# eleurent/rl-agents

Hardware: AMD Instinct MI355X
Metric: rollout env-steps/sec (UCT plan(), budget=1000) (higher is better)
Workload: dtype f64; 1 GPU; uct_highway_shaped_S10000_A5_budget1000_e33xh30_roots262144_per_gpu; n_roots_per_gpu=262144, n_roots_total=262144, states=10000, actions=5, episodes=33, horizon=30, parallelism=roots sharded over 1 GPU(s)

## Files before the change

rl_agents_amd/csrc/api.hip:

```cpp
#include <dlfcn.h>
#include <math.h>
#include <stdarg.h>
#include <stdlib.h>
#include <string.h>

#include <algorithm>
#include <mutex>
#include <set>
#include <unordered_map>
#include <vector>

#include "common.hpp"
#include "each_host.hpp"
#include "libm_sincos.hpp"
#include "seed_sequence.hpp"

namespace mp {

thread_local std::string g_err;

int fail(int code, const char *fmt, ...)
{
    char buf[1024];
    va_list ap;
    va_start(ap, fmt);
    vsnprintf(buf, sizeof(buf), fmt, ap);
    va_end(ap);
    g_err = buf;
    return code;
}

int ws_reserve(mp_ctx *ctx, int slot, size_t bytes, void **out)
{
    DevBuf &b = ctx->ws[slot];
    if (bytes > b.cap) {
        if (b.p) {
            MP_HIP(hipStreamSynchronize(ctx->stream));
            MP_HIP(hipFree(b.p));
// ... 102 lines not shown
    uint64_t k = (uint64_t)key;
    out[0] = (uint32_t)k;
    if (!(k >> 32)) return 1;
    out[1] = (uint32_t)(k >> 32);
    return 2;
}
}

__global__ void pack_records(int S, int A, const int32_t *__restrict__ T, const double *__restrict__ R,
                             const uint8_t *__restrict__ term, const uint8_t *__restrict__ avail, Rec *__restrict__ rec)
{
    const long i = (long)blockIdx.x * blockDim.x + threadIdx.x;
    if (i >= (long)S * A) return;
    const int s = (int)(i / A);
    Rec r;
    r.next = T[i];
    r.flags = (term && term[s] ? 1u : 0u) | (term && term[r.next] ? 2u : 0u) | (!avail || avail[i] ? 4u : 0u);
    r.reward = R[i];
    rec[i] = r;
}

__global__ void pack_records_range(int s0, int ns, int A, const int32_t *__restrict__ T, const double *__restrict__ R,
                                   const uint8_t *__restrict__ term, const uint8_t *__restrict__ avail, Rec *__restrict__ rec,
                                   uint16_t *__restrict__ t16)
{
    const long j = (long)blockIdx.x * blockDim.x + threadIdx.x;
    if (j >= (long)ns * A) return;
    const long i = (long)s0 * A + j;
    const int s = (int)(i / A);
    Rec r;
    r.next = T[i];
    r.flags = (term && term[s] ? 1u : 0u) | (term && term[r.next] ? 2u : 0u) | (!avail || avail[i] ? 4u : 0u);
    r.reward = R[i];
    rec[i] = r;
    if (t16) t16[i] = (uint16_t)((uint32_t)r.next | (term && term[r.next] ? 0x8000u : 0u));
}

__global__ void pack_joint_range(int first, int count, int M, int Sb, int A, long S, const int32_t *__restrict__ t_new,
                                 const double *__restrict__ r_new, const uint8_t *__restrict__ term_new,
                                 const uint8_t *__restrict__ avail, int32_t *__restrict__ T, double *__restrict__ R,
                                 uint8_t *__restrict__ term_all, Rec *__restrict__ rec_all)
{
    const long j = (long)blockIdx.x * blockDim.x + threadIdx.x;
    const long sa = (long)Sb * A;
    if (j >= (long)count * M * sa) return;
    const int cm = (int)(j / sa);
    const int c = cm / M, m = cm - c * M;
    const int sl = (int)((j - (long)cm * sa) / A), a = (int)(j - (long)cm * sa - (long)sl * A);
    const int base = (first + c) * Sb;
    const long i = ((long)m * S + base + sl) * A + a;
    const int nl = t_new[j];
    const uint8_t *tm = term_new ? term_new + (long)cm * Sb : nullptr;
    Rec r;
    r.next = base + nl;
    r.flags = (tm && tm[sl] ? 1u : 0u) | (tm && tm[nl] ? 2u : 0u) | (!avail || avail[i] ? 4u : 0u);
    r.reward = r_new[j];
    T[i] = r.next;
    R[i] = r.reward;
    rec_all[i] = r;
    if (a == 0 && tm) term_all[(long)m * S + base + sl] = tm[sl];
}

__global__ void scatter_rows(int n_rows, int A, const int32_t *__restrict__ rows, const int32_t *__restrict__ t_new,
                             const double *__restrict__ r_new, const uint8_t *__restrict__ term_new,
                             const uint8_t *__restrict__ r8_new, int32_t *__restrict__ T, double *__restrict__ R,
                             uint8_t *__restrict__ term, uint8_t *__restrict__ r8)
{
    const long j = (long)blockIdx.x * blockDim.x + threadIdx.x;
    if (j >= (long)n_rows * A) return;
    const int k = (int)(j / A), a = (int)(j - (long)k * A);
    const long i = (long)rows[k] * A + a;
    T[i] = t_new[j];
    R[i] = r_new[j];
    if (r8 && r8_new) r8[i] = r8_new[j];
    if (a == 0 && term && term_new) term[rows[k]] = term_new[k];
}

__global__ void pack_records_rows(int n_rows, int A, const int32_t *__restrict__ rows, const int32_t *__restrict__ T,
                                  const double *__restrict__ R, const uint8_t *__restrict__ term, const uint8_t *__restrict__ avail,
                                  Rec *__restrict__ rec, uint16_t *__restrict__ t16)
{
    const long j = (long)blockIdx.x * blockDim.x + threadIdx.x;
    if (j >= (long)n_rows * A) return;
    const int k = (int)(j / A), a = (int)(j - (long)k * A);
    const int s = rows[k];
    const long i = (long)s * A + a;
    Rec r;
    r.next = T[i];
    r.flags = (term && term[s] ? 1u : 0u) | (term && term[r.next] ? 2u : 0u) | (!avail || avail[i] ? 4u : 0u);
    r.reward = R[i];
    rec[i] = r;
    if (t16) t16[i] = (uint16_t)((uint32_t)r.next | (term && term[r.next] ? 0x8000u : 0u));
}

__global__ void globalize_roots(int n, int Sb, int NB, const int32_t *__restrict__ model_index, const int32_t *__restrict__ local,
                                int32_t *__restrict__ global, int32_t *__restrict__ fault)
{
    const int i = blockIdx.x * blockDim.x + threadIdx.x;
    if (i >= n) return;
    const int m = model_index[i], s = local[i];
    const bool bad = m < 0 || m >= NB || s < 0 || s >= Sb;
    if (bad && fault) atomicAdd(fault, 1);
    global[i] = bad ? 0 : m * Sb + s;
}

__global__ void globalize_joint_roots(int n, int M, int Sb, int NB, const int32_t *__restrict__ model_index,
                                      const int32_t *__restrict__ local, int32_t *__restrict__ global, int32_t *__restrict__ fault)
{
    const int i = blockIdx.x * blockDim.x + threadIdx.x;
    if (i >= n) return;
    const int b = model_index[i];
    bool bad = b < 0 || b >= NB;
    for (int m = 0; m < M; ++m) {
        const int s = local[(long)i * M + m];
        bad |= s < 0 || s >= Sb;
// ... 665 lines not shown
{
    const size_t n = (size_t)M * S * A;
    MP_HIP(hipSetDevice(ctx->device));
    mp_model *m = new mp_model();
    m->ctx = ctx; m->mode = MP_MODE_DETERMINISTIC; m->M = M; m->S = S; m->A = A; m->Sc = S; m->NB = 1; m->Sb = S;
    m->done_on_next = done_on_next ? 1 : 0; m->max_steps = max_steps > 0 ? max_steps : 0;
    auto bail = [&](int rc) { mp_model_free(m); return rc; };
    if (hipMalloc(&m->T, n * sizeof(int32_t)) != hipSuccess || hipMalloc(&m->R, n * sizeof(double)) != hipSuccess ||
        hipMalloc(&m->rec, (size_t)S * A * sizeof(Rec)) != hipSuccess)
        return bail(fail(MP_ERR_ALLOC, "mp_model_load_table: hipMalloc failed"));
    if (terminal && hipMalloc(&m->term, (size_t)S) != hipSuccess) return bail(fail(MP_ERR_ALLOC, "hipMalloc failed"));
    if (hipMemcpy(m->T, t32.data(), n * sizeof(int32_t), hipMemcpyHostToDevice) != hipSuccess ||
        hipMemcpy(m->R, reward, n * sizeof(double), hipMemcpyHostToDevice) != hipSuccess ||
        (terminal && hipMemcpy(m->term, terminal, (size_t)S, hipMemcpyHostToDevice) != hipSuccess))
        return bail(fail(MP_ERR_HIP, "mp_model_load_table: upload failed"));
    const long sa = (long)S * A;
    hipLaunchKernelGGL(pack_records, dim3((unsigned)((sa + 255) / 256)), dim3(256), 0, ctx->stream, S, A, m->T, m->R,
                       m->term, (const uint8_t *)nullptr, m->rec);
    if (S < 32768) {
        if (hipMalloc(&m->t16, (((size_t)sa * 2 + 15) & ~(size_t)15) + 16) != hipSuccess)
            return bail(fail(MP_ERR_ALLOC, "mp_model_load_table: hipMalloc failed"));
        hipLaunchKernelGGL(pack_t16, dim3((unsigned)((sa + 255) / 256)), dim3(256), 0, ctx->stream, S, A, m->T, m->term,
                           m->t16);
        m->rmap = new std::unordered_map<uint64_t, int>();
        std::unordered_map<uint64_t, int> &seen = *m->rmap;
        std::vector<uint8_t> idx(((size_t)sa + 15) & ~(size_t)15, 0);
        std::vector<double> dict(256, 0.0);
        bool fits = true;
        for (long i = 0; i < sa && fits; ++i) {
            uint64_t bits;
            memcpy(&bits, &reward[i], sizeof(bits));
            auto it = seen.find(bits);
            if (it == seen.end()) {
                if (seen.size() == 256) { fits = false; break; }
                it = seen.emplace(bits, (int)seen.size()).first;
                dict[it->second] = reward[i];
            }
            idx[i] = (uint8_t)it->second;
        }
        if (fits) {
            if (hipMalloc(&m->r8, idx.size()) != hipSuccess || hipMalloc(&m->rdict, 256 * sizeof(double)) != hipSuccess)
                return bail(fail(MP_ERR_ALLOC, "mp_model_load_table: hipMalloc failed"));
            if (hipMemcpy(m->r8, idx.data(), idx.size(), hipMemcpyHostToDevice) != hipSuccess ||
                hipMemcpy(m->rdict, dict.data(), 256 * sizeof(double), hipMemcpyHostToDevice) != hipSuccess)
                return bail(fail(MP_ERR_HIP, "mp_model_load_table: upload failed"));
            m->n_rdict = (int)seen.size();
// ... 151 lines not shown
        for (size_t i = 0; i < n && keep_compact; ++i) {
            const int k = reward_index(m, reward[i], &grew);
            if (k < 0) keep_compact = false;
            else idx[i] = (uint8_t)k;
        }
    }
    hipStream_t s = ctx->stream;
    const size_t g0 = (size_t)first * Sb;
    MP_HIP(hipMemcpyAsync(m->T + g0 * A, t32, n * 4, hipMemcpyHostToDevice, s));
    MP_HIP(hipMemcpyAsync(m->R + g0 * A, st + off_r, n * 8, hipMemcpyHostToDevice, s));
    if (terminal) MP_HIP(hipMemcpyAsync(m->term + g0, st + off_term, ns, hipMemcpyHostToDevice, s));
    if (compact && keep_compact) {
        MP_HIP(hipMemcpyAsync(m->r8 + g0 * A, st + off_r8, n, hipMemcpyHostToDevice, s));
        if (grew) {
            double *dict = reinterpret_cast<double *>(st + off_dict);
            for (const auto &kv : *m->rmap) memcpy(&dict[kv.second], &kv.first, 8);
            MP_HIP(hipMemcpyAsync(m->rdict, dict, m->rmap->size() * 8, hipMemcpyHostToDevice, s));
            m->n_rdict = (int)m->rmap->size();
        }
    } else if (compact) {
        drop_compact_rewards(m);
    }
    hipLaunchKernelGGL(pack_records_range, dim3((unsigned)((n + 255) / 256)), dim3(256), 0, s, (int)g0, (int)ns, A, m->T, m->R,
                       m->term, (const uint8_t *)m->avail, m->rec, m->t16);
    MP_HIP(hipGetLastError());
    MP_HIP(hipEventRecord(m->upd_done, s));
    m->upd_pending = true;
    m->serial = mp::next_model_serial();
    return MP_OK;
}

int mp_model_update_rows(mp_model *m, int32_t n_rows, const int32_t *rows, const int64_t *transition, const double *reward,
                         const uint8_t *terminal)
{
    if (!m || !rows || !transition || !reward) return fail(MP_ERR_ARG, "mp_model_update_rows: NULL argument");
    if (m->mode != MP_MODE_DETERMINISTIC || !m->rec || m->M != 1 || m->rec_all)
        return fail(MP_ERR_MODE, "mp_model_update_rows: deterministic table models (M = 1) only");
    if (n_rows < 1) return fail(MP_ERR_ARG, "mp_model_update_rows: n_rows = %d", n_rows);
    if (terminal && !m->term) return fail(MP_ERR_ARG, "mp_model_update_rows: the model was loaded without terminal flags");
    const int Sb = m->Sb > 0 ? m->Sb : m->S, A = m->A;
    mp_ctx *ctx = m->ctx;
    MP_HIP(hipSetDevice(ctx->device));
    const size_t n = (size_t)n_rows * A;
    const bool compact = m->r8 && m->rmap && m->n_rdict > 0;
    const size_t off_t = ((size_t)n_rows * 4 + 15) & ~(size_t)15, off_r = (off_t + n * 4 + 15) & ~(size_t)15, off_term = off_r + n * 8,
                 off_r8 = (off_term + n_rows + 15) & ~(size_t)15, off_dict = (off_r8 + n + 15) & ~(size_t)15, total = off_dict + 256 * 8;
    MP_TRY(update_blocks(m, total, total));
// ... 24 lines not shown
            else idx[i] = (uint8_t)k;
        }
    }
    if (compact && keep_compact && grew) {
        double *dict = reinterpret_cast<double *>(st + off_dict);
        for (const auto &kv : *m->rmap) memcpy(&dict[kv.second], &kv.first, 8);
    }
    hipStream_t s = ctx->stream;
    char *dv = static_cast<char *>(m->upd_dev);
    MP_HIP(hipMemcpyAsync(dv, st, total, hipMemcpyHostToDevice, s));
    if (compact && keep_compact && grew) {
        MP_HIP(hipMemcpyAsync(m->rdict, dv + off_dict, m->rmap->size() * 8, hipMemcpyDeviceToDevice, s));
        m->n_rdict = (int)m->rmap->size();
    }
    if (compact && !keep_compact) drop_compact_rewards(m);
    const int32_t *drows = reinterpret_cast<const int32_t *>(dv);
    hipLaunchKernelGGL(scatter_rows, dim3((unsigned)((n + 255) / 256)), dim3(256), 0, s, n_rows, A, drows,
                       reinterpret_cast<const int32_t *>(dv + off_t), reinterpret_cast<const double *>(dv + off_r),
                       terminal ? reinterpret_cast<const uint8_t *>(dv + off_term) : (const uint8_t *)nullptr,
                       compact && keep_compact ? reinterpret_cast<const uint8_t *>(dv + off_r8) : (const uint8_t *)nullptr, m->T, m->R,
                       m->term, compact && keep_compact ? m->r8 : (uint8_t *)nullptr);
    if (!terminal) {
        hipLaunchKernelGGL(pack_records_rows, dim3((unsigned)((n + 255) / 256)), dim3(256), 0, s, n_rows, A, drows, m->T, m->R, m->term,
                           (const uint8_t *)m->avail, m->rec, m->t16);
    } else {
        std::sort(owners.begin(), owners.end());
        owners.erase(std::unique(owners.begin(), owners.end()), owners.end());
        if (owners.size() > 64) {
            const long sa = (long)m->S * A;
            hipLaunchKernelGGL(pack_records_range, dim3((unsigned)((sa + 255) / 256)), dim3(256), 0, s, 0, m->S, A, m->T, m->R, m->term,
                               (const uint8_t *)m->avail, m->rec, m->t16);
        } else {
            const long sa = (long)Sb * A;
            for (int32_t b : owners)
                hipLaunchKernelGGL(pack_records_range, dim3((unsigned)((sa + 255) / 256)), dim3(256), 0, s, b * Sb, Sb, A, m->T, m->R,
                                   m->term, (const uint8_t *)m->avail, m->rec, m->t16);
        }
    }
    MP_HIP(hipGetLastError());
    MP_HIP(hipEventRecord(m->upd_done, s));
    m->upd_pending = true;
    m->serial = mp::next_model_serial();
    return MP_OK;
}

int mp_model_load_joint(mp_ctx *ctx, int32_t M, int32_t S, int32_t A, const int64_t *transition, const double *reward,
                        const uint8_t *terminal, int32_t done_on_next, mp_model **out)
{
    if (!ctx || !out || !transition || !reward) return fail(MP_ERR_ARG, "mp_model_load_joint: NULL argument");
    MP_TRY(mp_model_load_table(ctx, M, S, A, transition, reward, terminal, done_on_next, 0, out));
    mp_model *m = *out;
    auto bail = [&](int rc) { mp_model_free(m); *out = nullptr; return rc; };
    const long sa = (long)S * A;
    if (hipMalloc(&m->rec_all, (size_t)M * sa * sizeof(Rec)) != hipSuccess) return bail(fail(MP_ERR_ALLOC, "mp_model_load_joint: hipMalloc failed"));
    if (terminal) {
        if (hipMalloc(&m->term_all, (size_t)M * S) != hipSuccess) return bail(fail(MP_ERR_ALLOC, "mp_model_load_joint: hipMalloc failed"));
        if (hipMemcpy(m->term_all, terminal, (size_t)M * S, hipMemcpyHostToDevice) != hipSuccess)
            return bail(fail(MP_ERR_HIP, "mp_model_load_joint: upload failed"));
    }
// ... 313 lines not shown
    mp_model *m = new mp_model();
    m->ctx = ctx; m->mode = MP_MODE_CARTPOLE; m->M = 1; m->S = 0; m->A = 2;
    m->cp_sincos = mp_libm_sincos_variant();
    if (const char *e = getenv("MP_CARTPOLE_SINCOS"))
        m->cp_sincos = !strcmp(e, "fma") ? SINCOS_LIBM_FMA : (!strcmp(e, "plain") ? SINCOS_LIBM_PLAIN : SINCOS_DEVICE);
    m->cp = *params;
    m->max_steps = params->max_steps;
    *out = m;
    return MP_OK;
}

int mp_model_free(mp_model *m)
{
    if (!m) return MP_OK;
    if (m->ctx) hipSetDevice(m->ctx->device);
    if (!m->borrowed) {
        if (m->P) hipFree(const_cast<double *>(m->P));
        if (m->R) hipFree(m->R);
        if (m->term && m->term != m->term_all) hipFree(m->term);
    }
    if (m->T) hipFree(m->T);
    if (m->rec && m->rec != m->rec_all) hipFree(m->rec);
    if (m->t16) hipFree(m->t16);
    if (m->r8) hipFree(m->r8);
    if (m->rdict) hipFree(m->rdict);
    if (m->sa_cost) hipFree(m->sa_cost);
    if (m->avail) hipFree(m->avail);
    if (m->rec_all) hipFree(m->rec_all);
    if (m->term_all) hipFree(m->term_all);
    if (m->NXT) hipFree(m->NXT);
    if (m->thr) hipFree(m->thr);
    if (m->srec) hipFree(m->srec);
    if (m->srec_rtab) hipFree(m->srec_rtab);
    if (m->upd_pending && m->upd_done) (void)hipEventSynchronize(m->upd_done);
    if (m->upd_stage) (void)hipHostFree(m->upd_stage);
    if (m->upd_dev) hipFree(m->upd_dev);
    if (m->upd_done) (void)hipEventDestroy(m->upd_done);
    for (void *p : m->dead_blocks) (void)hipFree(p);
    delete m->rmap;
    delete m;
    return MP_OK;
}

int mp_model_info(const mp_model *m, int32_t *mode, int32_t *M, int32_t *S, int32_t *A, int32_t *B)
{
    if (!m) return fail(MP_ERR_ARG, "model is NULL");
// ... 30 lines not shown
```

rl_agents_amd/csrc/common.hpp:

```cpp
#pragma once
#include <hip/hip_runtime.h>
#include <stdint.h>
#include <stdio.h>
#include <string>
#include <unordered_map>
#include <vector>

#include "../../include/mi355plan.h"
#include "form_names.hpp"

namespace mp {

constexpr int kWave = 64;
constexpr size_t kLdsBytes = 160 * 1024;

extern thread_local std::string g_err;

int fail(int code, const char *fmt, ...);

#define MP_HIP(call)                                                                              \
    do {                                                                                          \
        hipError_t e_ = (call);                                                                   \
        if (e_ != hipSuccess)                                                                     \
            return mp::fail(MP_ERR_HIP, "%s failed: %s (%s:%d)", #call, hipGetErrorString(e_),    \
// ... 152 lines not shown
    int mode = 0, M = 1, S = 0, A = 0, B = 0;
    int Sc = 0;
    int NB = 1, Sb = 0;
    bool table_batch = false;
    void *upd_stage = nullptr;
    size_t upd_stage_cap = 0;
    void *upd_dev = nullptr;
    size_t upd_dev_cap = 0;
    hipEvent_t upd_done = nullptr;
    bool upd_pending = false;
    std::unordered_map<uint64_t, int> *rmap = nullptr;
    std::vector<void *> dead_blocks;
    int done_on_next = 0, max_steps = 0;
    bool masked = false;
    uint8_t *avail = nullptr;
    int32_t *T = nullptr;
    double *R = nullptr;
    uint8_t *term = nullptr;
    mp::Rec *rec = nullptr;
    mp::Rec *rec_all = nullptr;
    uint8_t *term_all = nullptr;
    bool joint_batch = false;
    uint16_t *t16 = nullptr;
    uint8_t *r8 = nullptr;
    double *rdict = nullptr;
    int n_rdict = 0;
    int32_t *sa_cost = nullptr;
    const double *P = nullptr;
    bool borrowed = false;
    int32_t *NXT = nullptr;
    uint64_t *thr = nullptr;
    uint4 *srec = nullptr;
    int srec_wb = 0;
    double *srec_rtab = nullptr;
    mp_cartpole_params cp;
    int cp_sincos = 0;
    int ss_w = 0;
    uint64_t ss_w_serial = 0;
};

struct mp_policy {
    mp_ctx *ctx = nullptr;
    const mp_model *model = nullptr;
    uint64_t model_serial = 0;
    int S = 0, A = 0;
    int stride = 0;
// ... 117 lines not shown
```

rl_agents_amd/csrc/pcg64.hpp:

```cpp
#pragma once
#include <stdint.h>
#if defined(__HIPCC__)
#include <hip/hip_runtime.h>
#define MP_PCG_FN __device__ __forceinline__
#else
#define MP_PCG_FN inline
#endif
#if defined(__has_builtin)
#if __has_builtin(__builtin_addc)
#define MP_PCG_HAS_ADDC 1
#endif
#endif

namespace mp {

#if defined(__HIPCC__)
struct Pcg64 {
    uint64_t s_hi, s_lo, inc_hi, inc_lo;
    uint32_t has_uint32, uinteger;

    __device__ __forceinline__ void load(const uint64_t *p)
    {
        s_hi = p[0]; s_lo = p[1]; inc_hi = p[2]; inc_lo = p[3] | 1ULL;
        has_uint32 = (uint32_t)p[4]; uinteger = (uint32_t)p[5];
    }
    __device__ __forceinline__ void store(uint64_t *p) const
    {
        p[0] = s_hi; p[1] = s_lo; p[2] = inc_hi; p[3] = inc_lo;
        p[4] = has_uint32; p[5] = uinteger;
    }
    __device__ __forceinline__ static uint64_t mad64(uint32_t a, uint32_t m, uint64_t c)
    {
        uint64_t d, cy;
        asm("v_mad_u64_u32 %0, %1, %2, %3, %4" : "=v"(d), "=s"(cy) : "v"(a), "s"(m), "v"(c));
// ... 224 lines not shown
        return (uint32_t)t;
#endif
    }
    template <typename G>
    MP_PCG_FN static Pcg64W from(const G &g)
    {
        Pcg64W w;
        w.w0 = (uint32_t)g.s_lo; w.w1 = (uint32_t)(g.s_lo >> 32); w.w2 = (uint32_t)g.s_hi; w.w3 = (uint32_t)(g.s_hi >> 32);
        w.i0 = (uint32_t)g.inc_lo; w.i1 = (uint32_t)(g.inc_lo >> 32); w.i2 = (uint32_t)g.inc_hi; w.i3 = (uint32_t)(g.inc_hi >> 32);
        return w;
    }
    template <typename G>
    MP_PCG_FN void state_to(G &g) const
    {
        g.s_lo = (uint64_t)w0 | ((uint64_t)w1 << 32);
        g.s_hi = (uint64_t)w2 | ((uint64_t)w3 << 32);
    }
    MP_PCG_FN void advance()
    {
        const uint32_t m0 = 0x9FCCF645u, m1 = 0x4385DF64u, m2 = 0x1FC65DA4u, m3 = 0x2360ED05u;
        const uint64_t A0 = mad64(w0, m0, 0);
        const uint64_t B = mad64(w0, m1, A0 >> 32);
        const uint64_t A1 = mad64(w1, m0, B);
        const uint32_t c1 = A1 < B ? 1u : 0u;
        const uint64_t C = mad64(w0, m2, A1 >> 32);
        const uint64_t D = mad64(w1, m1, C);
        const uint64_t A2 = mad64(w2, m0, D);
        uint64_t Q = mad64(w0, m3, 0);
        Q = mad64(w1, m2, Q);
        Q = mad64(w2, m1, Q);
        Q = mad64(w3, m0, Q);
        const uint32_t r1 = (uint32_t)A1, r3 = (uint32_t)Q + (uint32_t)(A2 >> 32) + c1;
        uint32_t r0 = (uint32_t)A0, r2 = (uint32_t)A2;
#if defined(__HIP_DEVICE_COMPILE__)
        asm volatile("" : "+v"(r0), "+v"(r2));
#endif
        uint32_t k;
        w0 = addc(r0, i0, 0u, &k);
        w1 = addc(r1, i1, k, &k);
        w2 = addc(r2, i2, k, &k);
        w3 = r3 + i3 + k;
    }
    MP_PCG_FN static uint32_t alignbit(uint32_t hi, uint32_t lo, uint32_t s)
    {
#if defined(__HIP_DEVICE_COMPILE__)
        return __builtin_amdgcn_alignbit(hi, lo, s);
#else
// ... 23 lines not shown
```

rl_agents_amd/csrc/uct.hip:

```cpp
#include <limits.h>
#include <math.h>
#include <stdlib.h>
#include <string.h>

#include <algorithm>
#include <new>
#include <vector>

#include <type_traits>

#include "common.hpp"
#include "libm_sincos.hpp"
#include "pcg64.hpp"
#include "uct_action_table.hpp"
#include "uct_balance.hpp"
#include "uct_host.hpp"
#include "uct_virgin.hpp"
#include "wave.hpp"

namespace mp {

struct alignas(16) UctNode {
    double value;
    int32_t count;
// ... 129 lines not shown
    return v;
}
#ifdef MP_WAVE_STAMPS
constexpr int kWaveStampWords = 8;
#endif

enum { ENV_TABLE = 0, ENV_CARTPOLE = 2, ENV_TABLE_LDSR = 3, ENV_TABLE_SPILL = 4 };

#ifndef MP_UCT_MIN_WAVES
#define MP_UCT_MIN_WAVES 1
#endif
#ifndef MP_PCG_WORDS
#define MP_PCG_WORDS 1
#endif
#ifndef MP_UCT_MASK_LOADS
#define MP_UCT_MASK_LOADS 1
#endif
#ifndef MP_UCT_READOUT_REGS
#define MP_UCT_READOUT_REGS 1
#endif
constexpr bool uct_pcg_words_form(int AT, int ENV, bool SP, bool MK, int IL, bool QD)
{
    return ENV != ENV_CARTPOLE && !QD;
}
template <int AT, int ENV, bool SP = false, bool MK = false, int IL = 0, bool QD = false, bool BAL = false, bool VM = false,
          bool ATAB = false>
__global__ __launch_bounds__(ENV == ENV_TABLE_LDSR ? 1024 : (ENV == ENV_CARTPOLE ? 256 : 64),
                             ENV == ENV_TABLE_LDSR ? 1 : (SP && AT > 0 && AT <= 5 && MP_UCT_MIN_WAVES < 4 ? 4 : MP_UCT_MIN_WAVES))
void uct_kernel(UctArgs p)
{
    static_assert(!SP || (AT > 0 && ENV == ENV_TABLE), "per-state policies: table env, |A| known at compile time");
    static_assert(!MK || SP, "listed policies are per-state policies");
    constexpr int NTH = AT > 1 ? AT - 1 : 1;
    constexpr int NQ = (NTH + 1) / 2;
    constexpr int NQ32 = (NTH + 3) / 4;
    constexpr bool LDSR = ENV == ENV_TABLE_LDSR;
    static_assert(!LDSR || (AT > 0 && !SP), "the LDS-resident variant: |A| at compile time, state-independent policies");
    static_assert(!QD || LDSR, "four lanes per root: the LDS-resident model");
    constexpr bool PREG = LDSR || ENV == ENV_TABLE_SPILL;
    constexpr bool CART = ENV == ENV_CARTPOLE;
    constexpr bool RAWU = AT > 0 && !SP;
    constexpr int USH = RAWU ? 0 : 11;
    static_assert(!BAL || (LDSR && !QD), "the wave balance: the one-lane LDS-resident form");
    extern __shared__ __attribute__((aligned(16))) double lds_raw[];
    extern __shared__ __attribute__((aligned(16))) uint32_t lds_bal[];
    static_assert(!ATAB || uct_action_table_form(AT, ENV, SP, MK, IL, QD), "the action table: the forms of uct_action_table_form");
// ... 85 lines not shown
    const TreeRef<IL, AT> tree = tree_of<IL, AT>(p.tree, r, p.cap, A);
    constexpr bool WEXP = IL == 2 && AT > 0 && AT <= 5 && !MK && !LDSR && !CART;
    constexpr int WEXP_PASSES = 4;
    constexpr bool LEAF1 = AT > 0 && !(LDSR && !QD && AT >= 7);
    const bool leaf1 = LEAF1 && p.tree_stores != 0;
    static_assert(!VM || (uct_mask_form(AT, ENV, SP, MK, IL, QD) && LEAF1 && !CART), "the visited mask: the forms of uct_mask_form");
    constexpr bool VMASK = VM;
    constexpr bool VSKIP = !VM && uct_virgin_form(AT, ENV, SP, MK, IL, QD);
    constexpr bool VDEFER = VSKIP && LEAF1;
    const bool vskip = VSKIP && p.tree_stores >= 2;
    const bool vdefer = VDEFER && p.tree_stores == 2 && p.n_nodes_in == nullptr;
    bool wave_exp = false;
    if constexpr (WEXP) {
        const int wave_r0 = (blockIdx.x * p.waves + __builtin_amdgcn_readfirstlane(wave)) * 64;
        wave_exp = p.tree_stores != 0 && p.lanes == 64 && wave_r0 + 64 <= p.n_roots;
    }
    const Rec *__restrict__ rec = p.rec;
    Pcg64 g;
    g.load(p.rng + (long)r * 6);
    constexpr bool PCGW = MP_PCG_WORDS != 0 && uct_pcg_words_form(AT, ENV, SP, MK, IL, QD);
    using RollGen = typename std::conditional<PCGW, Pcg64W, Pcg64>::type;
    auto roll_gen = [](const Pcg64 &x) { if constexpr (PCGW) return Pcg64W::from(x); else return x; };
    auto roll_gen_commit = [](Pcg64 &x, const RollGen &y) { if constexpr (PCGW) y.state_to(x); else x = y; };
    uint64_t g4_lo = 0, g4_hi = 0;
    if (QD || (CART && p.rep_shift >= 2)) g.inc_g4(g4_lo, g4_hi);
    uint64_t g16_lo = 0, g16_hi = 0;
    if (CART && p.rep_shift >= 4) g.inc_g16(g16_lo, g16_hi);
    const int32_t s0 = CART ? 0 : p.root_state[r];
    const int32_t st0 = p.root_steps ? p.root_steps[r] : 0;
    const uint32_t done_bit = p.done_on_next ? 2u : 1u;
    const bool root_term = CART ? false : (rec[(long)s0 * A].flags & 1u) != 0;
    double x0[4] = {0.0, 0.0, 0.0, 0.0};
    if (CART) {
#pragma unroll
        for (int i = 0; i < 4; ++i) x0[i] = p.root_x[(long)r * 4 + i];
    }
    const bool cart_flat = CART && p.cp_sincos != SINCOS_DEVICE && p.cp.theta_threshold < 0.8 && !any64(!(fabs(x0[2]) < 0.8));
    int n_nodes = p.n_nodes_in ? p.n_nodes_in[r] : 0;
    constexpr int AR = AT > 0 ? AT : 1;
    constexpr bool RC = AT > 0;
    double tv0 = 0.0, tv[AR];
    int tc0 = 0, tc[AR];
    int tf0 = -1, tf[AR];
#pragma unroll
    for (int a = 0; a < AR; ++a) { tv[a] = 0.0; tc[a] = 0; tf[a] = -1; }
    if (n_nodes < 1) {
// ... 46 lines not shown
        } else {                                                                                \
            int hh_ = pd_ == 0 ? tree.root_handle() : ph1;                                      \
            _Pragma("unroll") for (int i_ = 0; i_ < KEEP; ++i_) hh_ = pd_ == 2 + i_ ? ph[i_] : hh_; \
            if (pd_ >= 2 + KEEP) hh_ = p.path_spill[(size_t)pd_ * p.spill_stride + r];          \
            out_ = hh_;                                                                         \
        }                                                                                       \
    } while (0)

    constexpr int TREE_PRIO = LDSR && !QD ? 2 : 0;
#ifdef MP_PROFILE
    long long t_sel = 0, t_expd = 0, t_roll = 0, t_bak = 0, n_sel = 0, n_roll = 0;
    const long long t_all0 = clock64();
#define PROF_T(x) const long long x = clock64()
#else
#define PROF_T(x)
#endif
    for (int ep = 0; ep < E; ++ep) {
        PROF_T(c0);
        if constexpr (TREE_PRIO > 0) __builtin_amdgcn_s_setprio(TREE_PRIO);
        int32_t s = s0, st = st0;
        double x4[4] = {x0[0], x0[1], x0[2], x0[3]};
        int node = 0, depth = 0;
        bool terminal = false;
        bool cur_term = root_term;
        double total = 0.0;
        uint32_t cur_mask = mask0;
        if (!RC) PATH_PUT(0, tree.root_handle());
        int hnode = tree.root_handle();
        int fc = RC ? tf0 : tree[0].first_child;
        const bool beyond = RC && any64(tc0 >= TE);
        int node_c = 0;
        while (owner && depth < H && fc >= 0 && !terminal) {
            int act = 0, nfc = -1;
            if (AT > 0) {
                UctNode c[AR];
                bool virgin = false;
                const int fcw = fc;
                if (VMASK) fc &= kUctChildBits;
                if (fc == 1) {
#pragma unroll
                    for (int a = 0; a < AR; ++a) { c[a].value = tv[a]; c[a].count = tc[a]; c[a].first_child = tf[a]; }
                } else if (VMASK) {
                    UctNode *grp = &tree.child(fc, 0);
#pragma unroll
                    for (int a = 0; a < AR; ++a) {
                        const bool stored = ((fcw >> (kUctMaskShift + a)) & 1) != 0;
                        c[a].value = 0.0; c[a].count = 0; c[a].first_child = -1;
// ... 107 lines not shown
                int nt = 0;
                for (int a = 0; a < A; ++a) {
                    const UctNode c = tree.child(fc, a);
                    nt += (c.value + explore(a, c.count + 1)) == m ? 1 : 0;
                }
                int pick = (int)g.below((uint32_t)nt);
                for (int a = 0; a < A; ++a) {
                    const UctNode c = tree.child(fc, a);
                    if ((c.value + explore(a, c.count + 1)) == m) {
                        if (pick == 0) { act = a; nfc = c.first_child; break; }
                        --pick;
                    }
                }
            }
            const long idx = (long)s * A + act;
            double reward;
            if (CART) {
                terminal = cartpole_step(p.cp, x4, act, p.cp_sincos, sctab);
                reward = 1.0;
            } else if (LDSR) {
                const uint32_t e = t16[idx];
                reward = rdict[r8[idx]];
                const bool next_term = (e & 0x8000u) != 0;
                terminal = p.done_on_next ? next_term : cur_term;
                cur_term = next_term;
                s = (int32_t)(e & 0x7fffu);
            } else if (MK) {
                const uint4 q0 = p.pol_frec[(size_t)idx * (1 + NQ32)];
                terminal = (q0.y & done_bit) != 0;
                reward = __hiloint2double((int)q0.w, (int)q0.z);
                s = (int32_t)q0.x;
                cur_mask = (q0.y >> 8) & 0xffu;
            } else {
                const Rec rc = rec[idx];
                terminal = (rc.flags & done_bit) != 0;
                reward = rc.reward;
                s = rc.next;
            }
            ++st;
            ++steps_taken;
            total += gpow[depth] * reward;
            node = fc + act;
            hnode = tree.handle(fc, act);
            ++depth;
            PATH_PUT(depth, hnode);
            fc = nfc;
#ifdef MP_PROFILE
            ++n_sel;
// ... 434 lines not shown
                return t;
            };
            uint32_t act_next = 0;
            if constexpr (ATAB) act_next = table_action(u);
            bool stopped_in_a = true;
            double r_a = 0.0, r_b = 0.0, g_a = 0.0, g_b = 0.0;
            bool have_b = false;
            uint32_t tcur[NTH];
            if (SP) {
                const uint4 *tr = reinterpret_cast<const uint4 *>(p.pol_thr + (long)s * p.pol_stride);
                const int shift = p.pol_shift;
                const uint64_t sat = p.pol_sat;
                auto coarse = [shift, sat](uint32_t lo, uint32_t hi) {
                    const uint64_t c = (((uint64_t)hi << 32) | lo) >> shift;
                    return c > sat ? (uint32_t)sat : (uint32_t)c;
                };
#pragma unroll
                for (int q = 0; q < NQ; ++q) {
                    const uint4 v = tr[q];
                    if (2 * q < NTH) tcur[2 * q] = coarse(v.x, v.y);
                    if (2 * q + 1 < NTH) tcur[2 * q + 1] = coarse(v.z, v.w);
                }
            }
            auto step = [&](double &r_mine, double &g_mine, const double r_prev, const double g_prev, bool add_prev,
                            const RollGen &gcur, RollGen &gspec, uint64_t &unext) -> bool {
                int act = 0;
                if constexpr (ATAB) {
                    act = (int)act_next;
                } else
                if (SP) {
                    const uint32_t kh = (uint32_t)(u >> p.pol_shift);
                    bool ambiguous = false;
#pragma unroll
                    for (int a = 0; a < NTH; ++a) {
                        act += tcur[a] < kh ? 1 : 0;
                        ambiguous |= tcur[a] == kh;
                    }
                    if (ambiguous) {
                        const uint64_t *tx = p.pol_thr + (long)s * p.pol_stride;
                        act = 0;
#pragma unroll
                        for (int a = 0; a < NTH; ++a) act += tx[a] <= u ? 1 : 0;
                    }
                } else if (AT > 0) {
#pragma unroll
                    for (int a = 0; a < NTH; ++a) act += p.thr_arg[a] <= u ? 1 : 0;
                    act = min(act, p.thr_valid);
                } else {
                    for (int a = 0; a < A; ++a) act += thr[a] <= u ? 1 : 0;
                }
                g_mine = gpow[h];
                const unsigned ridx = PCGW && LDSR ? __umul24((unsigned)s, (unsigned)A) + (unsigned)act : (unsigned)(s * A + act);
                bool term_h;
                if (CART) {
                    gspec = gcur;
                    unext = gspec.next64() >> USH;
                    term_h = cartpole_step(p.cp, x4, act, p.cp_sincos, sctab);
                    total += g_mine * 1.0;
                } else if (LDSR) {
                    const unsigned idx = ridx;
                    const uint32_t e = t16[idx];
                    r_mine = rdict[r8[idx]];
                    gspec = gcur;
                    unext = gspec.next64() >> USH;
                    if constexpr (ATAB) act_next = table_action(unext);
                    total += g_prev * r_prev;
                    const bool next_term = (e & 0x8000u) != 0;
                    term_h = p.done_on_next ? next_term : cur_term;
                    cur_term = next_term;
                    s = (int32_t)(e & 0x7fffu);
                } else if (SP && NTH <= 4 && p.pol_packed) {
                    const uint4 q0 = p.pol_frec[ridx];
                    gspec = gcur;
                    unext = gspec.next64() >> USH;
                    term_h = (q0.y & done_bit) != 0;
                    s = (int32_t)(q0.x & 0xfffffu);
                    total += g_mine * __hiloint2double((int)q0.w, (int)q0.z);
                    tcur[0] = (q0.x >> 20) & 1023u;
                    if (NTH > 1) tcur[NTH > 1 ? 1 : 0] = (q0.y >> 2) & 1023u;
                    if (NTH > 2) tcur[NTH > 2 ? 2 : 0] = (q0.y >> 12) & 1023u;
                    if (NTH > 3) tcur[NTH > 3 ? 3 : 0] = (q0.y >> 22) & 1023u;
                } else if (SP) {
                    const uint4 *fr = p.pol_frec_roll + (size_t)ridx * (1 + NQ32);
                    const uint4 q0 = fr[0];
                    uint4 qt[NQ32];
#pragma unroll
                    for (int q = 0; q < NQ32; ++q) qt[q] = fr[1 + q];
                    gspec = gcur;
                    unext = gspec.next64() >> USH;
                    term_h = (q0.y & done_bit) != 0;
                    s = (int32_t)q0.x;
                    total += g_mine * __hiloint2double((int)q0.w, (int)q0.z);
#pragma unroll
                    for (int q = 0; q < NQ32; ++q) {
                        if (4 * q < NTH) tcur[4 * q] = qt[q].x;
                        if (4 * q + 1 < NTH) tcur[4 * q + 1] = qt[q].y;
                        if (4 * q + 2 < NTH) tcur[4 * q + 2] = qt[q].z;
                        if (4 * q + 3 < NTH) tcur[4 * q + 3] = qt[q].w;
                    }
                } else {
                    const Rec rc = rec[ridx];
                    gspec = gcur;
                    unext = gspec.next64() >> USH;
                    term_h = (rc.flags & done_bit) != 0;
                    s = rc.next;
                    total += g_mine * rc.reward;
                }
                ++h;
#ifdef MP_PROFILE
                ++n_roll;
#endif
                return term_h || h >= hmax;
            };
            while (true) {
                uint64_t un;
                if (step(r_a, g_a, r_b, g_b, have_b, ga, gb, un)) { stopped_in_a = true; break; }
                u = un;
                have_b = true;
                if (step(r_b, g_b, r_a, g_a, true, gb, ga, un)) { stopped_in_a = false; break; }
                u = un;
            }
            if (LDSR) total += stopped_in_a ? g_a * r_a : g_b * r_b;
            roll_gen_commit(g, stopped_in_a ? ga : gb);
            st += h - depth; steps_taken += h - depth;
        }
        if constexpr (TREE_PRIO > 0) __builtin_amdgcn_s_setprio(TREE_PRIO);
        PROF_T(c3);
        auto inv_fast = [&](int c) { if constexpr (RC) return inv_tab(c); else return inv(c); };
        typedef uint32_t stat3 __attribute__((ext_vector_type(3), may_alias));
        auto put_stats = [&](int n, double v, int cnt, bool leaf) {
            if (LEAF1 && leaf) {
                UctNode w;
                w.value = v; w.count = cnt; w.first_child = fc;
                tree.at(n) = w;
            } else {
                stat3 w;
                w.x = (uint32_t)__double2loint(v); w.y = (uint32_t)__double2hiint(v); w.z = (uint32_t)cnt;
                *reinterpret_cast<stat3 *>(&tree.at(n)) = w;
            }
        };
        bool leaf = leaf1;
        if (RC && beyond) {
            for (int d = depth; d >= 0; --d) {
                int n = 0;
// ... 1410 lines not shown
        memcpy(t.thr, a.thr_arg, sizeof(t.thr));
    }
    return t.bytes;
}

static int uct_form(mp_ctx *ctx, const UctPlan &c, bool cont, UctChoice *ch, UctArgs *a)
{
    const mp_model *model = c.model;
    UctCall call;
    call.n_roots = c.n_roots; call.episodes = c.episodes; call.horizon = c.horizon; call.A = model->A; call.S = model->S;
    call.NB = model->NB; call.Sb = model->Sb;
    call.t16 = model->t16 != nullptr; call.r8 = model->r8 != nullptr; call.n_rdict = model->n_rdict;
    call.cart = model->mode == MP_MODE_CARTPOLE; call.pol = c.pol != nullptr; call.listed = c.pol && c.pol->listed;
    call.kept_il = cont ? ctx->tree.il : -1;
    call.cus = ctx->prop.multiProcessorCount;
    const UctKnobs knobs = uct_knobs_read();
    MP_TRY(uct_choose(call, knobs, ch));
    a->tree_stores = knobs.tree_stores;
    a->balance = knobs.balance && ch->form == UF_LDSR && ch->lanes == 64 && ch->lds + kUctBalBytes <= kLdsBytes &&
                 model->A >= 2 && model->A <= 8 && uct_balance_form(model->A) ? 1 : 0;
    a->action_table = knobs.action_table && ch->form == UF_LDSR && ch->lanes == 64 && !c.pol &&
                      ch->lds + kUctBalBytes + kUctActBytes <= kLdsBytes &&
                      uct_action_table_form(model->A, ENV_TABLE_LDSR, false, false, ch->tree_il, false) ? 1 : 0;
    a->lanes = ch->lanes; a->waves = ch->waves; a->rep_shift = ch->rep_shift;
    a->jump = nullptr;
    const UctForm form = ch->form;
    if (form == UF_QUAD || form == UF_LONE || form == UF_LONE_MW || form == UF_LONE_EACH || form == UF_ROW_EACH || form == UF_ROW_SHARED ||
        form == UF_CARTPOLE)
        MP_TRY(uct_jump_table(ctx, c.horizon, &a->jump));
    return MP_OK;
}

static int uct_trees(mp_ctx *ctx, const UctPlan &c, bool cont, const UctChoice &ch, UctArgs *a)
{
    const int n_roots = c.n_roots, A = a->A, H = c.horizon, E = c.episodes;
    long cap_use = 1 + (long)E * A;
    a->n_nodes_in = nullptr;
    if (cont) {
        cap_use = uct_kept_cap(ctx, H, E, A);
        MP_TRY(uct_reroot_now(ctx, cap_use));
        MP_TRY(ws_get(ctx, WS_TREE1, (size_t)n_roots, &a->n_nodes_out));
        a->tree = (UctNode *)ctx->ws[ctx->tree.buf ? WS_TREE2 : WS_TREE0].p;
        a->n_nodes_in = a->n_nodes_out;
    } else {
        MP_TRY(ws_get(ctx, WS_TREE1, (size_t)n_roots, &a->n_nodes_out));
        uct_fresh_tree(ctx, H, E, A);
// ... 649 lines not shown
```

Before: 282.2 billion env-steps/s.

## Precompute source-terminal transition table and trim rollout step bookkeeping

Adds a second 16-bit transition table whose high bit holds the source state's terminal flag. Under the default not-done-on-next rule, the rollout loop can then read the terminal decision straight from the loaded word instead of carrying cur_term between steps. It also advances the horizon counter once per pair of unrolled steps, uses a cheaper comparison to test the terminal bit, and removes a carry compare in the PCG multiply, guarded by a static_assert on the multiplier. The cost is extra device memory, a host-side table build at load time, and extra writes in the record-update kernels.

```diff
diff --git a/rl_agents_amd/csrc/api.hip b/rl_agents_amd/csrc/api.hip
--- a/rl_agents_amd/csrc/api.hip
+++ b/rl_agents_amd/csrc/api.hip
@@ -14,6 +14,7 @@
 #include "each_host.hpp"
 #include "libm_sincos.hpp"
 #include "seed_sequence.hpp"
+#include "uct_term_table.hpp"
 
 namespace mp {
 
@@ -162,7 +163,7 @@
 
 __global__ void pack_records_range(int s0, int ns, int A, const int32_t *__restrict__ T, const double *__restrict__ R,
                                    const uint8_t *__restrict__ term, const uint8_t *__restrict__ avail, Rec *__restrict__ rec,
-                                   uint16_t *__restrict__ t16)
+                                   uint16_t *__restrict__ t16, uint16_t *__restrict__ t16s)
 {
     const long j = (long)blockIdx.x * blockDim.x + threadIdx.x;
     if (j >= (long)ns * A) return;
@@ -174,6 +175,7 @@
     r.reward = R[i];
     rec[i] = r;
     if (t16) t16[i] = (uint16_t)((uint32_t)r.next | (term && term[r.next] ? 0x8000u : 0u));
+    if (t16s) t16s[i] = uct_term_word(r.next, term && term[s], term && term[r.next], true);
 }
 
 __global__ void pack_joint_range(int first, int count, int M, int Sb, int A, long S, const int32_t *__restrict__ t_new,
@@ -218,7 +220,7 @@
 
 __global__ void pack_records_rows(int n_rows, int A, const int32_t *__restrict__ rows, const int32_t *__restrict__ T,
                                   const double *__restrict__ R, const uint8_t *__restrict__ term, const uint8_t *__restrict__ avail,
-                                  Rec *__restrict__ rec, uint16_t *__restrict__ t16)
+                                  Rec *__restrict__ rec, uint16_t *__restrict__ t16, uint16_t *__restrict__ t16s)
 {
     const long j = (long)blockIdx.x * blockDim.x + threadIdx.x;
     if (j >= (long)n_rows * A) return;
@@ -231,6 +233,7 @@
     r.reward = R[i];
     rec[i] = r;
     if (t16) t16[i] = (uint16_t)((uint32_t)r.next | (term && term[r.next] ? 0x8000u : 0u));
+    if (t16s) t16s[i] = uct_term_word(r.next, term && term[s], term && term[r.next], true);
 }
 
 __global__ void globalize_roots(int n, int Sb, int NB, const int32_t *__restrict__ model_index, const int32_t *__restrict__ local,
@@ -942,6 +945,15 @@
             return bail(fail(MP_ERR_ALLOC, "mp_model_load_table: hipMalloc failed"));
         hipLaunchKernelGGL(pack_t16, dim3((unsigned)((sa + 255) / 256)), dim3(256), 0, ctx->stream, S, A, m->T, m->term,
                            m->t16);
+        {
+            const size_t t16s_bytes = (((size_t)sa * 2 + 15) & ~(size_t)15) + 16;
+            std::vector<uint16_t> src_tab(t16s_bytes / 2, 0);
+            uct_term_table_fill(S, A, t32.data(), terminal, true, src_tab.data());
+            if (hipMalloc(&m->t16s, t16s_bytes) != hipSuccess)
+                return bail(fail(MP_ERR_ALLOC, "mp_model_load_table: hipMalloc failed"));
+            if (hipMemcpy(m->t16s, src_tab.data(), t16s_bytes, hipMemcpyHostToDevice) != hipSuccess)
+                return bail(fail(MP_ERR_HIP, "mp_model_load_table: upload failed"));
+        }
         m->rmap = new std::unordered_map<uint64_t, int>();
         std::unordered_map<uint64_t, int> &seen = *m->rmap;
         std::vector<uint8_t> idx(((size_t)sa + 15) & ~(size_t)15, 0);
@@ -1139,7 +1151,7 @@
         drop_compact_rewards(m);
     }
     hipLaunchKernelGGL(pack_records_range, dim3((unsigned)((n + 255) / 256)), dim3(256), 0, s, (int)g0, (int)ns, A, m->T, m->R,
-                       m->term, (const uint8_t *)m->avail, m->rec, m->t16);
+                       m->term, (const uint8_t *)m->avail, m->rec, m->t16, m->t16s);
     MP_HIP(hipGetLastError());
     MP_HIP(hipEventRecord(m->upd_done, s));
     m->upd_pending = true;
@@ -1210,19 +1222,19 @@
                        m->term, compact && keep_compact ? m->r8 : (uint8_t *)nullptr);
     if (!terminal) {
         hipLaunchKernelGGL(pack_records_rows, dim3((unsigned)((n + 255) / 256)), dim3(256), 0, s, n_rows, A, drows, m->T, m->R, m->term,
-                           (const uint8_t *)m->avail, m->rec, m->t16);
+                           (const uint8_t *)m->avail, m->rec, m->t16, m->t16s);
     } else {
         std::sort(owners.begin(), owners.end());
         owners.erase(std::unique(owners.begin(), owners.end()), owners.end());
         if (owners.size() > 64) {
             const long sa = (long)m->S * A;
             hipLaunchKernelGGL(pack_records_range, dim3((unsigned)((sa + 255) / 256)), dim3(256), 0, s, 0, m->S, A, m->T, m->R, m->term,
-                               (const uint8_t *)m->avail, m->rec, m->t16);
+                               (const uint8_t *)m->avail, m->rec, m->t16, m->t16s);
         } else {
             const long sa = (long)Sb * A;
             for (int32_t b : owners)
                 hipLaunchKernelGGL(pack_records_range, dim3((unsigned)((sa + 255) / 256)), dim3(256), 0, s, b * Sb, Sb, A, m->T, m->R,
-                                   m->term, (const uint8_t *)m->avail, m->rec, m->t16);
+                                   m->term, (const uint8_t *)m->avail, m->rec, m->t16, m->t16s);
         }
     }
     MP_HIP(hipGetLastError());
@@ -1582,6 +1594,7 @@
     if (m->T) hipFree(m->T);
     if (m->rec && m->rec != m->rec_all) hipFree(m->rec);
     if (m->t16) hipFree(m->t16);
+    if (m->t16s) hipFree(m->t16s);
     if (m->r8) hipFree(m->r8);
     if (m->rdict) hipFree(m->rdict);
     if (m->sa_cost) hipFree(m->sa_cost);
diff --git a/rl_agents_amd/csrc/common.hpp b/rl_agents_amd/csrc/common.hpp
--- a/rl_agents_amd/csrc/common.hpp
+++ b/rl_agents_amd/csrc/common.hpp
@@ -198,6 +198,7 @@
     uint8_t *term_all = nullptr;
     bool joint_batch = false;
     uint16_t *t16 = nullptr;
+    uint16_t *t16s = nullptr;
     uint8_t *r8 = nullptr;
     double *rdict = nullptr;
     int n_rdict = 0;
diff --git a/rl_agents_amd/csrc/pcg64.hpp b/rl_agents_amd/csrc/pcg64.hpp
--- a/rl_agents_amd/csrc/pcg64.hpp
+++ b/rl_agents_amd/csrc/pcg64.hpp
@@ -10,6 +10,9 @@
 #if __has_builtin(__builtin_addc)
 #define MP_PCG_HAS_ADDC 1
 #endif
+#endif
+#ifndef MP_PCG_NO_C1
+#define MP_PCG_NO_C1 1
 #endif
 
 namespace mp {
@@ -280,7 +283,12 @@
         const uint64_t A0 = mad64(w0, m0, 0);
         const uint64_t B = mad64(w0, m1, A0 >> 32);
         const uint64_t A1 = mad64(w1, m0, B);
+#if MP_PCG_NO_C1
+        static_assert((uint64_t)m0 + (uint64_t)m1 < (1ULL << 32), "Pcg64W: column 1 can carry for this multiplier, keep the compare");
+        const uint32_t c1 = 0u;
+#else
         const uint32_t c1 = A1 < B ? 1u : 0u;
+#endif
         const uint64_t C = mad64(w0, m2, A1 >> 32);
         const uint64_t D = mad64(w1, m1, C);
         const uint64_t A2 = mad64(w2, m0, D);
diff --git a/rl_agents_amd/csrc/uct.hip b/rl_agents_amd/csrc/uct.hip
--- a/rl_agents_amd/csrc/uct.hip
+++ b/rl_agents_amd/csrc/uct.hip
@@ -175,6 +175,19 @@
 constexpr bool uct_pcg_words_form(int AT, int ENV, bool SP, bool MK, int IL, bool QD)
 {
     return ENV != ENV_CARTPOLE && !QD;
+}
+#ifndef MP_UCT_TERM_TABLE
+#define MP_UCT_TERM_TABLE 1
+#endif
+#ifndef MP_UCT_LEAN_INDEX
+#define MP_UCT_LEAN_INDEX 1
+#endif
+#ifndef MP_UCT_LEAN_COUNT
+#define MP_UCT_LEAN_COUNT 1
+#endif
+constexpr bool uct_term_table_form(int ENV, bool QD)
+{
+    return MP_UCT_TERM_TABLE != 0 && ENV == ENV_TABLE_LDSR && !QD;
 }
 template <int AT, int ENV, bool SP = false, bool MK = false, int IL = 0, bool QD = false, bool BAL = false, bool VM = false,
           bool ATAB = false>
@@ -306,6 +319,9 @@
     using RollGen = typename std::conditional<PCGW, Pcg64W, Pcg64>::type;
     auto roll_gen = [](const Pcg64 &x) { if constexpr (PCGW) return Pcg64W::from(x); else return x; };
     auto roll_gen_commit = [](Pcg64 &x, const RollGen &y) { if constexpr (PCGW) y.state_to(x); else x = y; };
+    constexpr bool TERMTAB = uct_term_table_form(ENV, QD);
+    constexpr bool LEANI = MP_UCT_LEAN_INDEX != 0 && PCGW && LDSR;
+    constexpr bool LEANH = MP_UCT_LEAN_COUNT != 0 && PCGW;
     uint64_t g4_lo = 0, g4_hi = 0;
     if (QD || (CART && p.rep_shift >= 2)) g.inc_g4(g4_lo, g4_hi);
     uint64_t g16_lo = 0, g16_hi = 0;
@@ -398,7 +414,7 @@
         double x4[4] = {x0[0], x0[1], x0[2], x0[3]};
         int node = 0, depth = 0;
         bool terminal = false;
-        bool cur_term = root_term;
+        [[maybe_unused]] bool cur_term = root_term;
         double total = 0.0;
         uint32_t cur_mask = mask0;
         if (!RC) PATH_PUT(0, tree.root_handle());
@@ -552,8 +568,12 @@
                 const uint32_t e = t16[idx];
                 reward = rdict[r8[idx]];
                 const bool next_term = (e & 0x8000u) != 0;
-                terminal = p.done_on_next ? next_term : cur_term;
-                cur_term = next_term;
+                if constexpr (TERMTAB) {
+                    terminal = next_term;
+                } else {
+                    terminal = p.done_on_next ? next_term : cur_term;
+                    cur_term = next_term;
+                }
                 s = (int32_t)(e & 0x7fffu);
             } else if (MK) {
                 const uint4 q0 = p.pol_frec[(size_t)idx * (1 + NQ32)];
@@ -1034,8 +1054,9 @@
                     if (2 * q + 1 < NTH) tcur[2 * q + 1] = coarse(v.z, v.w);
                 }
             }
-            auto step = [&](double &r_mine, double &g_mine, const double r_prev, const double g_prev, bool add_prev,
+            auto step = [&](auto second_tag, double &r_mine, double &g_mine, const double r_prev, const double g_prev, bool add_prev,
                             const RollGen &gcur, RollGen &gspec, uint64_t &unext) -> bool {
+                constexpr int SECOND = decltype(second_tag)::value ? 1 : 0;
                 int act = 0;
                 if constexpr (ATAB) {
                     act = (int)act_next;
@@ -1061,7 +1082,7 @@
                 } else {
                     for (int a = 0; a < A; ++a) act += thr[a] <= u ? 1 : 0;
                 }
-                g_mine = gpow[h];
+                g_mine = LEANH ? gpow[h - 2 + SECOND] : gpow[h];
                 const unsigned ridx = PCGW && LDSR ? __umul24((unsigned)s, (unsigned)A) + (unsigned)act : (unsigned)(s * A + act);
                 bool term_h;
                 if (CART) {
@@ -1071,15 +1092,20 @@
                     total += g_mine * 1.0;
                 } else if (LDSR) {
                     const unsigned idx = ridx;
-                    const uint32_t e = t16[idx];
+                    uint32_t e = t16[idx];
+                    if constexpr (LEANI) asm("" : "+v"(e));
                     r_mine = rdict[r8[idx]];
                     gspec = gcur;
                     unext = gspec.next64() >> USH;
                     if constexpr (ATAB) act_next = table_action(unext);
                     total += g_prev * r_prev;
-                    const bool next_term = (e & 0x8000u) != 0;
-                    term_h = p.done_on_next ? next_term : cur_term;
-                    cur_term = next_term;
+                    const bool next_term = LEANI ? e > 0x7fffu : (e & 0x8000u) != 0;
+                    if constexpr (TERMTAB) {
+                        term_h = next_term;
+                    } else {
+                        term_h = p.done_on_next ? next_term : cur_term;
+                        cur_term = next_term;
+                    }
                     s = (int32_t)(e & 0x7fffu);
                 } else if (SP && NTH <= 4 && p.pol_packed) {
                     const uint4 q0 = p.pol_frec[ridx];
@@ -1118,20 +1144,26 @@
                     s = rc.next;
                     total += g_mine * rc.reward;
                 }
-                ++h;
 #ifdef MP_PROFILE
                 ++n_roll;
 #endif
-                return term_h || h >= hmax;
+                if constexpr (LEANH) {
+                    return term_h || (SECOND ? h >= hmax : h > hmax);
+                } else {
+                    ++h;
+                    return term_h || h >= hmax;
+                }
             };
             while (true) {
                 uint64_t un;
-                if (step(r_a, g_a, r_b, g_b, have_b, ga, gb, un)) { stopped_in_a = true; break; }
+                if constexpr (LEANH) h += 2;
+                if (step(std::false_type{}, r_a, g_a, r_b, g_b, have_b, ga, gb, un)) { stopped_in_a = true; break; }
                 u = un;
                 have_b = true;
-                if (step(r_b, g_b, r_a, g_a, true, gb, ga, un)) { stopped_in_a = false; break; }
+                if (step(std::true_type{}, r_b, g_b, r_a, g_a, true, gb, ga, un)) { stopped_in_a = false; break; }
                 u = un;
             }
+            if constexpr (LEANH) h -= stopped_in_a ? 1 : 0;
             if (LDSR) total += stopped_in_a ? g_a * r_a : g_b * r_b;
             roll_gen_commit(g, stopped_in_a ? ga : gb);
             st += h - depth; steps_taken += h - depth;
@@ -2588,6 +2620,10 @@
     a->action_table = knobs.action_table && ch->form == UF_LDSR && ch->lanes == 64 && !c.pol &&
                       ch->lds + kUctBalBytes + kUctActBytes <= kLdsBytes &&
                       uct_action_table_form(model->A, ENV_TABLE_LDSR, false, false, ch->tree_il, false) ? 1 : 0;
+    if (uct_term_table_form(ENV_TABLE_LDSR, false) && ch->form == UF_LDSR && !model->done_on_next) {
+        if (!model->t16s) return fail(MP_ERR_ARG, "mp_uct_plan: the model has no source-rule transition table");
+        a->t16 = model->t16s;
+    }
     a->lanes = ch->lanes; a->waves = ch->waves; a->rep_shift = ch->rep_shift;
     a->jump = nullptr;
     const UctForm form = ch->form;
diff --git a/rl_agents_amd/csrc/uct_term_table.hpp b/rl_agents_amd/csrc/uct_term_table.hpp
--- /dev/null
+++ b/rl_agents_amd/csrc/uct_term_table.hpp
@@ -0,0 +1,27 @@
+#pragma once
+
+#include <cstdint>
+
+#if defined(__HIPCC__)
+#define MP_TERM_TABLE_FN __host__ __device__ inline
+#else
+#define MP_TERM_TABLE_FN inline
+#endif
+
+namespace mp {
+
+MP_TERM_TABLE_FN uint16_t uct_term_word(int32_t next, bool term_s, bool term_next, bool source)
+{
+    return (uint16_t)((uint32_t)next | ((source ? term_s : term_next) ? 0x8000u : 0u));
+}
+
+inline void uct_term_table_fill(int S, int A, const int32_t *T, const uint8_t *term, bool source, uint16_t *out)
+{
+    for (int s = 0; s < S; ++s)
+        for (int a = 0; a < A; ++a) {
+            const int32_t nx = T[(long)s * A + a];
+            out[(long)s * A + a] = uct_term_word(nx, term && term[s], term && term[nx], source);
+        }
+}
+
+}
```

After: 298.9 billion env-steps/s (median of 6 runs). 5.9% higher.
